# JuliaLinearAlgebra/IterativeSolvers.jl

Hardware: AMD Instinct MI355X
Metric: cg_iters_per_sec (higher is better)
Workload: dtype f64; 1 GPU; cg! on 256^3 3D 7-point Laplacian (test/laplace_matrix.jl), fp64, hashed rhs, x0 = 0 (BASELINE.json configs[1]); n=16777216, nnz=117047296

## Files before the change

iterativesolvers.jl_amd/csrc/mik_iter.h:

```cpp
#pragma once
#include "mik_internal.h"

template <typename T> struct CgDev {
    T res, prev_res, alpha, beta, dot_uc, rr, tol, rho;
    T beta_rho;
    int done, nhist;
    int x_pending, pad_;
};

struct CgMirror {
    double res, prev_res, tol;
    int done, nhist;
    int tol_valid;
    int range;
    unsigned long long seq;
};

struct mik_cg {
    mik_ctx *ctx = nullptr;
    const mik_csr *A = nullptr;
    int dtype = MIK_F64;
    int64_t n = 0;
    void *x = nullptr, *u = nullptr, *r = nullptr, *c = nullptr;
    const void *b = nullptr, *diag = nullptr;
    mik_mul_fn op_mul = nullptr;
    void *op_user = nullptr;
    mik_ldiv_fn pl_fn = nullptr;
    void *pl_user = nullptr;
    void *dev = nullptr;
    void *fin = nullptr;
    void *hist = nullptr;
    int64_t hist_cap = 0;
    void *seg_spmv = nullptr;
    void *seg_vec = nullptr;
    void *seg_vec2 = nullptr;
    bool pcg_fused = false;
    double residual = 0, prev_residual = 1, tol = 0;
    int64_t maxiter = 0, mv_products = 0;
    CgMirror *mirror = nullptr;
    unsigned long long seq = 0;
    bool dev_done = false;
    bool head_ahead = false;
    bool fuse_x = false;
    int profile = 0;
    std::vector<hipEvent_t> ev;
    std::vector<int> ev_kind;
    size_t ev_used = 0;
    double kern_ms[3] = {0, 0, 0};
    int64_t kern_launches[3] = {0, 0, 0};
};

#ifdef __HIPCC__
constexpr int MIK_FIN_WGS = MIK_FIN_THREADS / 64;
template <typename T> struct FinScratch { T ws[MIK_FIN_WGS]; unsigned ticket; };

template <typename T> __device__ __forceinline__ bool level2_sum_spread(const T *__restrict__ S, int64_t m, FinScratch<T> *fs, T &tot)
{
    const int w = blockIdx.x, lane = threadIdx.x;
    T acc = T(0);
    int64_t j = 64 * (int64_t)w + lane;
    for (; j + 63 * (int64_t)MIK_FIN_THREADS < m; j += 64 * (int64_t)MIK_FIN_THREADS) {
        T v[64];
#pragma unroll
        for (int q = 0; q < 64; ++q) v[q] = S[j + q * (int64_t)MIK_FIN_THREADS];
#pragma unroll
        for (int q = 0; q < 64; ++q) acc = acc + v[q];
    }
    for (; j + 15 * (int64_t)MIK_FIN_THREADS < m; j += 16 * (int64_t)MIK_FIN_THREADS) {
        T v[16];
#pragma unroll
        for (int q = 0; q < 16; ++q) v[q] = S[j + q * (int64_t)MIK_FIN_THREADS];
#pragma unroll
        for (int q = 0; q < 16; ++q) acc = acc + v[q];
    }
    for (; j + 7 * (int64_t)MIK_FIN_THREADS < m; j += 8 * (int64_t)MIK_FIN_THREADS) {
        T v[8];
#pragma unroll
        for (int q = 0; q < 8; ++q) v[q] = S[j + q * (int64_t)MIK_FIN_THREADS];
#pragma unroll
        for (int q = 0; q < 8; ++q) acc = acc + v[q];
    }
    for (; j < m; j += MIK_FIN_THREADS) acc = acc + S[j];
    acc = wave_tree(acc);
    bool last = false;
    if (lane == 0) {
        __hip_atomic_store(&fs->ws[w], acc, __ATOMIC_RELAXED, __HIP_MEMORY_SCOPE_AGENT);
        asm volatile("s_waitcnt vmcnt(0)" ::: "memory");
        const unsigned tk = __hip_atomic_fetch_add(&fs->ticket, 1u, __ATOMIC_RELAXED, __HIP_MEMORY_SCOPE_AGENT);
        if (tk == (unsigned)gridDim.x - 1u) {
            T t = __hip_atomic_load(&fs->ws[0], __ATOMIC_RELAXED, __HIP_MEMORY_SCOPE_AGENT);
#pragma unroll
            for (int q = 1; q < MIK_FIN_WGS; ++q) t = t + __hip_atomic_load(&fs->ws[q], __ATOMIC_RELAXED, __HIP_MEMORY_SCOPE_AGENT);
            __hip_atomic_store(&fs->ticket, 0u, __ATOMIC_RELAXED, __HIP_MEMORY_SCOPE_AGENT);
            tot = t;
            last = true;
        }
    }
    return last;
}

template <typename T>
__device__ __forceinline__ void cgd_close_step(CgDev<T> *d, T tot, T *__restrict__ hist, long long it_next, long long maxiter, CgMirror *mirror,
                                               unsigned long long seq, int hist_index, int fuse_x)
{
    if (fuse_x) d->x_pending = 1;
    if (!mik_nrm_in_range(tot)) {
        d->done = 1; mirror->done = 0; mirror->nhist = hist_index; mirror->range = 1;
        __hip_atomic_store(&mirror->seq, seq, __ATOMIC_RELEASE, __HIP_MEMORY_SCOPE_SYSTEM);
        return;
    }
    const T prev = d->res;
    const T res = mik_sqrt(tot);
    d->rr = tot; d->prev_res = prev; d->res = res;
    d->beta = (res * res) / (prev * prev);
    hist[hist_index] = res;
    const int nh = hist_index + 1;
    const int dn = (it_next >= maxiter || res <= d->tol) ? 1 : 0;
    if (dn) d->done = 1;
    mirror->res = (double)res; mirror->prev_res = (double)prev; mirror->done = dn; mirror->nhist = nh;
    __hip_atomic_store(&mirror->seq, seq, __ATOMIC_RELEASE, __HIP_MEMORY_SCOPE_SYSTEM);
}
#endif

int cg_wait_mirror(mik_cg *it);

template <class R> static int cg_run_batch(R &rk, int64_t iteration, int64_t max_steps, bool ahead_ok, double *residuals, int64_t *steps_done)
// ... 83 lines not shown
```

iterativesolvers.jl_amd/csrc/mik_kernels.h:

```cpp
#pragma once
#include <algorithm>

#include "mik_internal.h"

#ifdef __HIPCC__


template <typename T, bool VEC, typename Op>
__global__ __launch_bounds__(MIK_BLOCK) void k_map(int64_t n, int64_t nseg, Op op, T *__restrict__ seg_out,
                                                    const int *__restrict__ done)
{
    if (done && *done) return;
    constexpr int W = VT<T>::W;
    constexpr int L = MIK_RED_L;
    constexpr int64_t SEG = (int64_t)MIK_BLOCK * W * L;
    __shared__ T lds4[4];
    for (int64_t s = blockIdx.x; s < nseg; s += gridDim.x) {
        const int64_t base = s * SEG + (int64_t)W * threadIdx.x;
        T acc = T(0);
#pragma unroll
        for (int l = 0; l < L; ++l) {
            const int64_t i = base + (int64_t)l * MIK_BLOCK * W;
            if (VEC && i + W <= n) {
                op.apply_vec(i, acc);
// ... 469 lines not shown
        auto xv = vload<T>(x + i); auto yv = vload<T>(y + i);
#pragma unroll
        for (int e = 0; e < VT<T>::W; ++e) { el<T>(xv, e) = el<T>(xv, e) * a; el<T>(yv, e) = el<T>(yv, e) * b; }
        vstore(x + i, xv); vstore(y + i, yv);
    }
};

template <typename T> struct OpQmrUpdate {
    static constexpr bool REDUCE = false;
    const T *__restrict__ v; const T *p_curr; const T *p_prev; T *p_out; T *__restrict__ x; T neg_h1, neg_h0, inv, g;
    __device__ __forceinline__ void apply(int64_t i, T &) const
    {
        T p = v[i];
        if (p_curr) { T t = neg_h1 * p_curr[i]; p = p + t; }
        if (p_prev) { T t = neg_h0 * p_prev[i]; p = p + t; }
        p = p * inv;
        p_out[i] = p;
        T t = g * p; x[i] = x[i] + t;
    }
    __device__ __forceinline__ void apply_vec(int64_t i, T &) const
    {
        constexpr int W = VT<T>::W;
        auto pv = vload(v + i); auto xv = vload_nt<T>(x + i);
        if (p_curr) {
            auto cv = vload(p_curr + i);
#pragma unroll
            for (int e = 0; e < W; ++e) { T t = neg_h1 * el<T>(cv, e); el<T>(pv, e) = el<T>(pv, e) + t; }
        }
        if (p_prev) {
            auto qv = vload(p_prev + i);
#pragma unroll
            for (int e = 0; e < W; ++e) { T t = neg_h0 * el<T>(qv, e); el<T>(pv, e) = el<T>(pv, e) + t; }
        }
#pragma unroll
        for (int e = 0; e < W; ++e) { el<T>(pv, e) = el<T>(pv, e) * inv; T t = g * el<T>(pv, e); el<T>(xv, e) = el<T>(xv, e) + t; }
        vstore(p_out + i, pv); vstore_nt(x + i, xv);
    }
};

template <typename T> struct OpXpbyX {
    static constexpr bool REDUCE = false;
    const T *__restrict__ r; T *__restrict__ u; T *__restrict__ x; Coef<T> beta, alpha;
    const int *__restrict__ done; const int *__restrict__ pending; int nt = 0;
    __device__ __forceinline__ void apply(int64_t i, T &) const
    {
        const int dn = *done, pd = *pending;
        if (dn && !pd) return;
        const T uo = u[i];
        if (pd) { T t = alpha.get() * uo; x[i] = x[i] + t; }
        if (!dn) { T t = beta.get() * uo; u[i] = r[i] + t; }
    }
    __device__ __forceinline__ void apply_vec(int64_t i, T &) const
    {
        const int dn = *done, pd = *pending;
        if (dn && !pd) return;
        auto uv = (nt & 2) ? vload_nt<T>(u + i) : vload<T>(u + i);
        if (pd) {
            const T a = alpha.get();
            auto xv = (nt & 8) ? vload_nt<T>(x + i) : vload<T>(x + i);
#pragma unroll
            for (int e = 0; e < VT<T>::W; ++e) { T t = a * el<T>(uv, e); el<T>(xv, e) = el<T>(xv, e) + t; }
            if (nt & 8) vstore_nt(x + i, xv); else vstore(x + i, xv);
        }
        if (!dn) {
            const T b = beta.get();
            auto rv = (nt & 1) ? vload_nt(r + i) : vload(r + i);
#pragma unroll
            for (int e = 0; e < VT<T>::W; ++e) { T t = b * el<T>(uv, e); el<T>(uv, e) = el<T>(rv, e) + t; }
            if (nt & 4) vstore_nt(u + i, uv); else vstore(u + i, uv);
        }
    }
};

template <typename T> struct CoefAlphaRanks {
    const T *all; int nranks; const T *res;
    __device__ __forceinline__ T get() const
    {
        T tot = all[0];
        for (int p = 1; p < nranks; ++p) tot = tot + all[p];
        const T r = *res;
        return (r * r) / tot;
    }
};
template <typename T, typename C = Coef<T>> struct OpCgUpdateR {
    static constexpr bool REDUCE = true;
    T *__restrict__ r; const T *__restrict__ c; C alpha; int nt = 0;
    __device__ __forceinline__ void apply(int64_t i, T &acc) const
    {
        T s = alpha.get() * c[i]; T rn = r[i] - s; r[i] = rn;
        T p = rn * rn; acc = acc + p;
    }
    __device__ __forceinline__ void apply_vec(int64_t i, T &acc) const
    {
        const T a = alpha.get();
        auto rv = (nt & 8) ? vload_nt<T>(r + i) : vload<T>(r + i);
        auto cv = (nt & 2) ? vload_nt(c + i) : vload(c + i);
#pragma unroll
        for (int e = 0; e < VT<T>::W; ++e) { T s = a * el<T>(cv, e); el<T>(rv, e) = el<T>(rv, e) - s; }
        if (nt & 16) vstore_nt(r + i, rv); else vstore(r + i, rv);
#pragma unroll
        for (int e = 0; e < VT<T>::W; ++e) { T p = el<T>(rv, e) * el<T>(rv, e); acc = acc + p; }
    }
};

template <typename T> struct OpPcgUpdateR {
    static constexpr bool REDUCE = true;
    T *__restrict__ r; T *__restrict__ c; const T *__restrict__ d; Coef<T> alpha; int nt = 0;
    __device__ __forceinline__ void apply(int64_t i, T &a1, T &a2) const
    {
        T s = alpha.get() * c[i]; T rn = r[i] - s; r[i] = rn;
        T p = rn * rn; a1 = a1 + p;
        T v = rn / d[i]; c[i] = v;
        T q = v * rn; a2 = a2 + q;
    }
    __device__ __forceinline__ void apply_vec(int64_t i, T &a1, T &a2) const
    {
        const T a = alpha.get();
        auto rv = (nt & 8) ? vload_nt<T>(r + i) : vload<T>(r + i);
        auto cv = (nt & 64) ? vload_nt<T>(c + i) : vload<T>(c + i);
        auto dv = vload_nt(d + i);
#pragma unroll
        for (int e = 0; e < VT<T>::W; ++e) { T s = a * el<T>(cv, e); el<T>(rv, e) = el<T>(rv, e) - s; }
        if (nt & 16) vstore_nt(r + i, rv); else vstore(r + i, rv);
#pragma unroll
        for (int e = 0; e < VT<T>::W; ++e) { T p = el<T>(rv, e) * el<T>(rv, e); a1 = a1 + p; }
#pragma unroll
        for (int e = 0; e < VT<T>::W; ++e) el<T>(cv, e) = el<T>(rv, e) / el<T>(dv, e);
        if (nt & 32) vstore_nt(c + i, cv); else vstore(c + i, cv);
#pragma unroll
        for (int e = 0; e < VT<T>::W; ++e) { T q = el<T>(cv, e) * el<T>(rv, e); a2 = a2 + q; }
    }
};

template <typename T> struct OpXFlush {
    static constexpr bool REDUCE = false;
    const T *__restrict__ u; T *__restrict__ x; Coef<T> alpha; const int *__restrict__ pending;
    __device__ __forceinline__ void apply(int64_t i, T &) const
    {
        if (!*pending) return;
        T t = alpha.get() * u[i]; x[i] = x[i] + t;
    }
    __device__ __forceinline__ void apply_vec(int64_t i, T &) const
    {
        if (!*pending) return;
        const T a = alpha.get();
        auto uv = vload(u + i); auto xv = vload<T>(x + i);
#pragma unroll
        for (int e = 0; e < VT<T>::W; ++e) { T t = a * el<T>(uv, e); el<T>(xv, e) = el<T>(xv, e) + t; }
        vstore(x + i, xv);
    }
};

template <typename T> struct OpAxpy {
    static constexpr bool REDUCE = false;
    const T *__restrict__ x; T *__restrict__ y; Coef<T> alpha;
    __device__ __forceinline__ void apply(int64_t i, T &) const { T t = alpha.get() * x[i]; y[i] = y[i] + t; }
    __device__ __forceinline__ void apply_vec(int64_t i, T &) const
    {
        const T a = alpha.get();
        auto xv = vload(x + i); auto yv = vload<T>(y + i);
#pragma unroll
        for (int e = 0; e < VT<T>::W; ++e) { T t = a * el<T>(xv, e); el<T>(yv, e) = el<T>(yv, e) + t; }
        vstore(y + i, yv);
    }
};

template <typename T> struct OpBicgU {
    static constexpr bool REDUCE = false;
    T *__restrict__ us; int64_t ldu; const T *__restrict__ rs; int64_t ldr; int ncols; Coef<T> neg_beta;
    int nt = 0;
    __device__ __forceinline__ void apply(int64_t i, T &) const
    {
        const T b = neg_beta.get();
        for (int q = 0; q < ncols; ++q) { T *u = us + q * ldu; T t = b * u[i]; u[i] = rs[q * ldr + i] + t; }
    }
    __device__ __forceinline__ void apply_vec(int64_t i, T &) const
    {
        const T b = neg_beta.get();
        for (int q = 0; q < ncols; ++q) {
            T *u = us + q * ldu;
            auto xv = (nt & 1) ? vload_nt(rs + q * ldr + i) : vload(rs + q * ldr + i);
            auto yv = (nt & 1) ? vload_nt<T>(u + i) : vload<T>(u + i);
#pragma unroll
            for (int e = 0; e < VT<T>::W; ++e) { T t = b * el<T>(yv, e); el<T>(yv, e) = el<T>(xv, e) + t; }
            if (q + 1 < ncols ? (nt & 2) : (nt & 4)) vstore_nt(u + i, yv); else vstore(u + i, yv);
        }
// ... 988 lines not shown
```

iterativesolvers.jl_amd/csrc/mik_krylov.hip:

```cpp
#include <algorithm>
#include <cfloat>
#include <cstddef>
#include <cmath>
#include <map>
#include <new>
#include <tuple>

#include "mik_kernels.h"
#include "mik_mgs_res.h"
#include "mik_iter.h"
#include "mik_mail.h"

template <typename T>
int mik_spmv_launch(mik_ctx *ctx, const mik_csr *A, const T *x, T *y, bool fuse_dot, T *seg_out, const int *done);
template <typename T>
int mik_spmv_launch_range(mik_ctx *ctx, const mik_csr *A, const T *x, T *y, bool fuse_dot, T *seg_out, const int *done, int rb_begin,
                          int rb_count);
template <typename T>
int mik_spmv_launch_outside(mik_ctx *ctx, const mik_csr *A, const T *x, T *y, bool fuse_dot, T *seg_out, const int *done, int skip_begin, int skip_end);
bool mik_spmv_can_split(const mik_csr *A);
bool mik_spmv_is_light(const mik_csr *A);



// ... 377 lines not shown
        for (int q = 0; q < 16; ++q) { a1 = a1 + v[q]; a2 = a2 + z[q]; }
    }
    for (; j < m; j += MIK_FIN_THREADS) { a1 = a1 + S1[j]; a2 = a2 + S2[j]; }
    a1 = wave_tree(a1);
    a2 = wave_tree(a2);
    bool last = false;
    if (lane == 0) {
        __hip_atomic_store(&fs->ws[w], a1, __ATOMIC_RELAXED, __HIP_MEMORY_SCOPE_AGENT);
        __hip_atomic_store(&fs->ws2[w], a2, __ATOMIC_RELAXED, __HIP_MEMORY_SCOPE_AGENT);
        asm volatile("s_waitcnt vmcnt(0)" ::: "memory");
        const unsigned tk = __hip_atomic_fetch_add(&fs->ticket, 1u, __ATOMIC_RELAXED, __HIP_MEMORY_SCOPE_AGENT);
        if (tk == (unsigned)gridDim.x - 1u) {
            T t = __hip_atomic_load(&fs->ws[0], __ATOMIC_RELAXED, __HIP_MEMORY_SCOPE_AGENT);
            T z = __hip_atomic_load(&fs->ws2[0], __ATOMIC_RELAXED, __HIP_MEMORY_SCOPE_AGENT);
#pragma unroll
            for (int q = 1; q < MIK_FIN_WGS; ++q) {
                t = t + __hip_atomic_load(&fs->ws[q], __ATOMIC_RELAXED, __HIP_MEMORY_SCOPE_AGENT);
                z = z + __hip_atomic_load(&fs->ws2[q], __ATOMIC_RELAXED, __HIP_MEMORY_SCOPE_AGENT);
            }
            __hip_atomic_store(&fs->ticket, 0u, __ATOMIC_RELAXED, __HIP_MEMORY_SCOPE_AGENT);
            tot1 = t; tot2 = z;
            last = true;
        }
    }
    return last;
}

template <typename T> __device__ __forceinline__ void cg_init_scalars(CgDev<T> *d, T tot, T res, T reltol, T abstol, long long maxiter)
{
    const T a = reltol * res;
    d->rr = tot;
    d->res = res;
    d->prev_res = T(1);
    d->rho = T(1);
    d->tol = a > abstol ? a : abstol;
    d->beta = (res * res) / (T(1) * T(1));
    d->alpha = T(0);
    d->dot_uc = T(0);
    d->done = (0 >= maxiter || res <= d->tol) ? 1 : 0;
    d->nhist = 0;
}

template <typename T>
__global__ __launch_bounds__(MIK_FIN_THREADS) void k_cg_fin_init(const T *__restrict__ S, int64_t m, CgDev<T> *d, T reltol, T abstol,
                                                                 long long maxiter)
{
    __shared__ T lds16[16];
    T tot = level2_sum(S, m, lds16);
    if (threadIdx.x == 0) { cg_init_scalars(d, tot, mik_sqrt(tot), reltol, abstol, maxiter); d->x_pending = 0; }
}

template <typename T> __global__ void k_cg_set_init(CgDev<T> *d, T res, T reltol, T abstol, long long maxiter)
{
    cg_init_scalars(d, res * res, res, reltol, abstol, maxiter);
    d->x_pending = 0;
}

template <typename T>
__global__ __launch_bounds__(64) void k_cg_fin_alpha(const T *__restrict__ S, int64_t m, CgDev<T> *d, int pcg, FinScratch<T> *fs)
{
    if (blockIdx.x == 0 && threadIdx.x == 0) d->x_pending = 0;
    if (d->done) return;
    T tot;
    if (level2_sum_spread(S, m, fs, tot)) {
        d->dot_uc = tot;
        const T num = pcg ? d->rho : d->res * d->res;
        d->alpha = num / tot;
    }
}

template <typename T>
__global__ __launch_bounds__(64) void k_cg_fin_rho(const T *__restrict__ S, int64_t m, CgDev<T> *d, FinScratch<T> *fs)
{
    if (d->done) return;
    T tot;
    if (level2_sum_spread(S, m, fs, tot)) {
        const T rho_prev = d->rho;
        d->rho = tot;
        d->beta = tot / rho_prev;
    }
}

template <typename T>
__device__ __forceinline__ void cg_res_scalars(CgDev<T> *d, T tot, T res, T *__restrict__ hist, long long it_next, long long maxiter,
                                               CgMirror *mirror, unsigned long long seq, int hist_index, int pcg_fused = 0)
{
    const T prev = d->res;
    d->rr = tot;
    d->prev_res = prev;
    d->res = res;
    d->beta = pcg_fused ? d->beta_rho : (res * res) / (prev * prev);
    hist[hist_index] = res;
    const int dn = (it_next >= maxiter || res <= d->tol) ? 1 : 0;
    if (dn) d->done = 1;
    mirror->res = (double)res;
    mirror->prev_res = (double)prev;
    mirror->done = dn;
    mirror->nhist = hist_index + 1;
    __hip_atomic_store(&mirror->seq, seq, __ATOMIC_RELEASE, __HIP_MEMORY_SCOPE_SYSTEM);
}

template <typename T>
__global__ __launch_bounds__(64) void k_cg_fin_res(const T *__restrict__ S, int64_t m, CgDev<T> *d, T *__restrict__ hist,
                                                    long long it_next, long long maxiter, CgMirror *mirror,
                                                    unsigned long long seq, int hist_index, FinScratch<T> *fs, int fuse_x)
{
    if (d->done) {
        if (blockIdx.x == 0 && threadIdx.x == 0) __hip_atomic_store(&mirror->seq, seq, __ATOMIC_RELEASE, __HIP_MEMORY_SCOPE_SYSTEM);
        return;
    }
    T tot;
    if (level2_sum_spread(S, m, fs, tot)) {
        if (fuse_x) d->x_pending = 1;
        if (!mik_nrm_in_range(tot)) {
            d->done = 1;
            mirror->done = 0;
            mirror->nhist = hist_index;
            mirror->range = 1;
            __hip_atomic_store(&mirror->seq, seq, __ATOMIC_RELEASE, __HIP_MEMORY_SCOPE_SYSTEM);
            return;
        }
        cg_res_scalars(d, tot, mik_sqrt(tot), hist, it_next, maxiter, mirror, seq, hist_index);
    }
}

template <typename T>
__global__ void k_cg_fix_res(CgDev<T> *d, T res, T *__restrict__ hist, long long it_next, long long maxiter, CgMirror *mirror,
                             unsigned long long seq, int hist_index, int pcg_fused = 0)
{
    d->done = 0;
    mirror->range = 0;
    cg_res_scalars(d, res * res, res, hist, it_next, maxiter, mirror, seq, hist_index, pcg_fused);
}

template <typename T>
__global__ __launch_bounds__(64) void k_cg_fin_res2(const T *__restrict__ S1, const T *__restrict__ S2, int64_t m, CgDev<T> *d, T *__restrict__ hist,
                                                     long long it_next, long long maxiter, CgMirror *mirror, unsigned long long seq, int hist_index,
                                                     FinScratch2<T> *fs)
{
    if (d->done) {
        if (blockIdx.x == 0 && threadIdx.x == 0) __hip_atomic_store(&mirror->seq, seq, __ATOMIC_RELEASE, __HIP_MEMORY_SCOPE_SYSTEM);
        return;
    }
    T tot, tot2;
    if (level2_sum_spread2(S1, S2, m, fs, tot, tot2)) {
        d->x_pending = 1;
        const T rho_prev = d->rho;
        d->rho = tot2;
        d->beta_rho = tot2 / rho_prev;
        if (!mik_nrm_in_range(tot)) {
            d->done = 1;
            mirror->done = 0;
            mirror->nhist = hist_index;
            mirror->range = 1;
            __hip_atomic_store(&mirror->seq, seq, __ATOMIC_RELEASE, __HIP_MEMORY_SCOPE_SYSTEM);
            return;
        }
        cg_res_scalars(d, tot, mik_sqrt(tot), hist, it_next, maxiter, mirror, seq, hist_index, 1);
    }
}

static int cg_profile_collect(mik_cg *it)
{
    size_t i = 0;
    for (; i + 1 < it->ev_used; i += 2) {
        if (hipEventQuery(it->ev[i + 1]) != hipSuccess) { (void)hipGetLastError(); break; }
        float ms = 0.f;
        const int kind = it->ev_kind[i / 2];
        if (hipEventElapsedTime(&ms, it->ev[i], it->ev[i + 1]) == hipSuccess) { it->kern_ms[kind] += ms; it->kern_launches[kind] += 1; }
    }
    size_t keep = 0;
    for (size_t j = i; j + 1 < it->ev_used; j += 2, keep += 2) {
        std::swap(it->ev[keep], it->ev[j]);
        std::swap(it->ev[keep + 1], it->ev[j + 1]);
        it->ev_kind[keep / 2] = it->ev_kind[j / 2];
    }
    it->ev_used = keep;
    return MIK_OK;
}

static void cg_profile_flush(mik_cg *it)
{
    if (!it->ev_used) return;
    (void)hipStreamSynchronize(it->ctx->stream);
    (void)cg_profile_collect(it);
}

struct CgProfileScope {
    mik_cg *it; bool on;
    CgProfileScope(mik_cg *it_, int kind) : it(it_), on(it_->profile == 2 || (it_->profile == 1 && kind == 0))
    {
        if (!on) return;
        if (it->ev_used + 2 > it->ev.size()) {
            hipEvent_t a, b;
            if (hipEventCreate(&a) != hipSuccess || hipEventCreate(&b) != hipSuccess) { on = false; return; }
            it->ev.push_back(a); it->ev.push_back(b);
            it->ev_kind.push_back(0);
        }
        it->ev_kind[it->ev_used / 2] = kind;
        (void)hipEventRecord(it->ev[it->ev_used], it->ctx->stream);
    }
    ~CgProfileScope()
    {
        if (!on) return;
        (void)hipEventRecord(it->ev[it->ev_used + 1], it->ctx->stream);
        it->ev_used += 2;
    }
};

static inline int cg_stream_hints(const mik_ctx *ctx, bool fused_x = false, const mik_csr *A = nullptr)
{
    (void)ctx;
    return fused_x ? (mik_spmv_is_light(A) ? 248 : 121) : 57;
}


static inline int cg_sweep_u_hints(const mik_cg *it) { return it->fuse_x ? cg_stream_hints(it->ctx, true, it->A) & 15 : cg_stream_hints(it->ctx) & 7; }

template <typename T> static int cg_sweep_u(mik_cg *it, const T *src, int64_t lo, int64_t len, bool vec, int hints)
{
    CgDev<T> *d = (CgDev<T> *)it->dev;
    T *x = (T *)it->x, *u = (T *)it->u;
    if (it->fuse_x) {
        OpXpbyX<T> op{src + lo, u + lo, x + lo, coef_ptr<T>(&d->beta), coef_ptr<T>(&d->alpha), &d->done, &d->x_pending, hints};
        return launch_map<T>(it->ctx, len, op, vec, (T *)nullptr, (const int *)nullptr);
    }
    OpXpby<T> op{src + lo, u + lo, coef_ptr<T>(&d->beta), hints};
    return launch_map<T>(it->ctx, len, op, vec, (T *)nullptr, &d->done);
}

template <typename T, typename C> static int cg_update_xr(mik_cg *it, C alpha, bool vec)
{
    CgDev<T> *d = (CgDev<T> *)it->dev;
    T *x = (T *)it->x, *u = (T *)it->u, *r = (T *)it->r, *c = (T *)it->c;
    if (it->fuse_x) {
        OpCgUpdateR<T, C> up{r, c, alpha, cg_stream_hints(it->ctx, true, it->A) >> 3};
        return launch_map<T>(it->ctx, it->n, up, vec, (T *)it->seg_vec, &d->done);
    }
    if constexpr (std::is_same<C, Coef<T>>::value) {
        OpCgUpdate<T> up{x, r, u, c, alpha, cg_stream_hints(it->ctx) >> 3};
        return launch_map<T>(it->ctx, it->n, up, vec, (T *)it->seg_vec, &d->done);
    }
    return mik_fail(it->ctx, MIK_ERR_INVALID, "cg: alpha formed inside the sweep needs the x update on the next sweep over u");
}

template <typename T> __global__ void k_cg_clear_pending(CgDev<T> *d) { d->x_pending = 0; }

template <typename T> static int cg_flush_x(mik_cg *it)
{
    mik_ctx *ctx = it->ctx;
    CgDev<T> *d = (CgDev<T> *)it->dev;
    T *x = (T *)it->x, *u = (T *)it->u;
    OpXFlush<T> op{u, x, coef_ptr<T>(&d->alpha), &d->x_pending};
    MIK_TRY((launch_map<T>(ctx, it->n, op, mik_aligned16(x) && mik_aligned16(u), (T *)nullptr, (const int *)nullptr)));
    hipLaunchKernelGGL((k_cg_clear_pending<T>), dim3(1), dim3(1), 0, ctx->stream, d);
    MIK_LAUNCH_CHECK(ctx);
    return MIK_OK;
}

template <typename T> static int cg_init_residual(mik_cg *it, const T *x0, bool vec)
{
    mik_ctx *ctx = it->ctx;
    T *c = (T *)it->c;
    it->mv_products = x0 ? 1 : 0;
    if (x0) {
        if (it->A) MIK_TRY(mik_spmv_launch<T>(ctx, it->A, x0, c, false, nullptr, nullptr));
        else if (it->op_mul(it->op_user, x0, c) != 0) return mik_fail(ctx, MIK_ERR_CALLBACK, "cg: the operator callback failed");
    }
    OpSubNrm<T> op{(const T *)it->b, x0 ? c : nullptr, (T *)it->r};
    return launch_map<T>(ctx, it->n, op, vec, (T *)it->seg_vec, nullptr);
}

template <typename T> static int cg_enqueue_head(mik_cg *it)
{
    mik_ctx *ctx = it->ctx;
    CgDev<T> *d = (CgDev<T> *)it->dev;
    const int *done = &d->done;
    const int64_t n = it->n, nseg = mik_nseg<T>(n);
    T *x = (T *)it->x, *u = (T *)it->u, *r = (T *)it->r, *c = (T *)it->c;
    const bool vec = mik_aligned16(x) && mik_aligned16(u) && mik_aligned16(r) && mik_aligned16(c) && (!it->diag || mik_aligned16(it->diag));
    const int pcg = (it->diag || it->pl_fn) ? 1 : 0;
    if (it->pcg_fused) {
    } else if (it->diag) {
        OpJacobiDot<T> pj{r, (const T *)it->diag, c, cg_stream_hints(ctx) != 0};
        MIK_TRY((launch_map<T>(ctx, n, pj, vec, (T *)it->seg_vec, done)));
    } else if (it->pl_fn) {
        if (it->pl_fn(it->pl_user, c, r) != 0) return mik_fail(ctx, MIK_ERR_CALLBACK, "cg: the preconditioner callback failed");
        OpDot<T> dcr{c, r};
        MIK_TRY((launch_map<T>(ctx, n, dcr, vec, (T *)it->seg_vec, done)));
    }
    if (pcg && !it->pcg_fused) {
        hipLaunchKernelGGL((k_cg_fin_rho<T>), dim3(MIK_FIN_WGS), dim3(64), 0, ctx->stream, (const T *)it->seg_vec, nseg, d, (FinScratch<T> *)it->fin);
        MIK_LAUNCH_CHECK(ctx);
    }
    {
        CgProfileScope ps(it, 1);
        const int pcg_hints = it->fuse_x ? (cg_stream_hints(ctx, true, it->A) & 8) | 1 : cg_stream_hints(ctx) & 1;
        MIK_TRY(cg_sweep_u<T>(it, pcg ? c : r, 0, n, vec, pcg ? pcg_hints : cg_sweep_u_hints(it)));
    }
    if (it->A) {
        CgProfileScope ps(it, 0);
        MIK_TRY(mik_spmv_launch<T>(ctx, it->A, u, c, true, (T *)it->seg_spmv, done));
    } else {
        if (it->op_mul(it->op_user, u, c) != 0) return mik_fail(ctx, MIK_ERR_CALLBACK, "cg: the operator callback failed");
        OpDot<T> duc{u, c};
        MIK_TRY((launch_map<T>(ctx, n, duc, vec, (T *)it->seg_vec, done)));
    }
    hipLaunchKernelGGL((k_cg_fin_alpha<T>), dim3(MIK_FIN_WGS), dim3(64), 0, ctx->stream, (const T *)(it->A ? it->seg_spmv : it->seg_vec), it->A ? mik_spmv_nwg(n) : nseg,
                       d, pcg, (FinScratch<T> *)it->fin);
    MIK_LAUNCH_CHECK(ctx);
    return MIK_OK;
}

template <typename T> static int cg_enqueue_tail(mik_cg *it, long long it_next, int hist_index)
{
    mik_ctx *ctx = it->ctx;
    CgDev<T> *d = (CgDev<T> *)it->dev;
    const int *done = &d->done;
    const int64_t n = it->n, nseg = mik_nseg<T>(n);
    T *x = (T *)it->x, *u = (T *)it->u, *r = (T *)it->r, *c = (T *)it->c;
    const bool vec = mik_aligned16(x) && mik_aligned16(u) && mik_aligned16(r) && mik_aligned16(c) && (!it->diag || mik_aligned16(it->diag));
    if (it->pcg_fused) {
        {
            CgProfileScope ps(it, 2);
            OpPcgUpdateR<T> up{r, c, (const T *)it->diag, coef_ptr<T>(&d->alpha), 120};
            MIK_TRY((launch_map2<T>(ctx, n, up, vec, (T *)it->seg_vec, (T *)it->seg_vec2, done)));
        }
        it->seq += 1;
        hipLaunchKernelGGL((k_cg_fin_res2<T>), dim3(MIK_FIN_WGS), dim3(64), 0, ctx->stream, (const T *)it->seg_vec, (const T *)it->seg_vec2, nseg, d, (T *)it->hist,
                           it_next, (long long)it->maxiter, it->mirror, it->seq, hist_index, (FinScratch2<T> *)((unsigned char *)it->fin + 512));
        MIK_LAUNCH_CHECK(ctx);
        return MIK_OK;
    }
    {
        CgProfileScope ps(it, 2);
        MIK_TRY(cg_update_xr<T>(it, coef_ptr<T>(&d->alpha), vec));
    }
    it->seq += 1;
    hipLaunchKernelGGL((k_cg_fin_res<T>), dim3(MIK_FIN_WGS), dim3(64), 0, ctx->stream, (const T *)it->seg_vec, nseg, d, (T *)it->hist,
                       it_next, (long long)it->maxiter, it->mirror, it->seq, hist_index, (FinScratch<T> *)it->fin, it->fuse_x ? 1 : 0);
    MIK_LAUNCH_CHECK(ctx);
    return MIK_OK;
}

int cg_wait_mirror(mik_cg *it)
{
    volatile unsigned long long *p = &it->mirror->seq;
    const unsigned long long want = it->seq;
    for (unsigned long long spins = 0;; ++spins) {
        if (__atomic_load_n((const unsigned long long *)p, __ATOMIC_ACQUIRE) == want) return MIK_OK;
        if ((spins & 0xFFFFF) == 0xFFFFF) {
            hipError_t e = hipStreamQuery(it->ctx->stream);
            if (e == hipSuccess) {
                if (__atomic_load_n((const unsigned long long *)p, __ATOMIC_ACQUIRE) == want) return MIK_OK;
                return mik_fail(it->ctx, MIK_ERR_HIP, "cg: stream idle but step %llu was never published", want);
            }
            if (e != hipErrorNotReady) return mik_fail(it->ctx, MIK_ERR_HIP, "cg: %s while waiting for a step", hipGetErrorString(e));
        }
#if defined(__x86_64__)
        __builtin_ia32_pause();
#endif
    }
}

template <typename T> static int cg_fetch_state(mik_cg *it, CgDev<T> *host)
{
    mik_ctx *ctx = it->ctx;
    MIK_HIP(ctx, hipMemcpyAsync(ctx->coef_host, it->dev, sizeof(CgDev<T>), hipMemcpyDeviceToHost, ctx->stream));
    MIK_HIP(ctx, hipStreamSynchronize(ctx->stream));
    memcpy(host, ctx->coef_host, sizeof(CgDev<T>));
    return MIK_OK;
}

template <typename T>
static int cg_init_impl(mik_cg *it, double abstol, double reltol, int initially_zero)
{
    mik_ctx *ctx = it->ctx;
    const int64_t n = it->n, nseg = mik_nseg<T>(n);
    T *u = (T *)it->u, *r = (T *)it->r, *c = (T *)it->c;
    OpFill<T> z{u, T(0)};
    MIK_TRY((launch_map<T>(ctx, n, z, mik_aligned16(u), (T *)nullptr, nullptr)));
    const bool vec = mik_aligned16(r) && mik_aligned16(it->b) && mik_aligned16(c);
    MIK_TRY(cg_init_residual<T>(it, initially_zero ? nullptr : (const T *)it->x, vec));
    hipLaunchKernelGGL((k_cg_fin_init<T>), dim3(1), dim3(MIK_FIN_THREADS), 0, ctx->stream, (const T *)it->seg_vec, nseg,
                       (CgDev<T> *)it->dev, (T)reltol, (T)abstol, (long long)it->maxiter);
    MIK_LAUNCH_CHECK(ctx);
    CgDev<T> h;
    MIK_TRY(cg_fetch_state<T>(it, &h));
    if (!mik_nrm_in_range(h.rr)) {
        T res;
        MIK_TRY(mik_safe_norm_slow<T>(ctx, n, r, &res));
        hipLaunchKernelGGL((k_cg_set_init<T>), dim3(1), dim3(1), 0, ctx->stream, (CgDev<T> *)it->dev, res, (T)reltol, (T)abstol, (long long)it->maxiter);
        MIK_LAUNCH_CHECK(ctx);
        MIK_TRY(cg_fetch_state<T>(it, &h));
    }
    it->residual = (double)h.res;
    it->prev_residual = (double)h.prev_res;
    it->tol = (double)h.tol;
    it->dev_done = h.done != 0;
    if (it->pcg_fused) {
        OpJacobiDot<T> pj{r, (const T *)it->diag, c, 0};
        MIK_TRY((launch_map<T>(ctx, n, pj, vec && mik_aligned16(it->diag), (T *)it->seg_vec, (const int *)nullptr)));
        hipLaunchKernelGGL((k_cg_fin_rho<T>), dim3(MIK_FIN_WGS), dim3(64), 0, ctx->stream, (const T *)it->seg_vec, nseg, (CgDev<T> *)it->dev, (FinScratch<T> *)it->fin);
        MIK_LAUNCH_CHECK(ctx);
    }
    return MIK_OK;
}

static int cg_create_common(mik_ctx *ctx, const mik_csr *A, int dtype, int64_t n, mik_mul_fn op_mul, void *op_user, const void *jacobi_diag,
                            mik_ldiv_fn pl_fn, void *pl_user, void *x, const void *b, void *u, void *r, void *c, double abstol, double reltol,
                            int64_t maxiter, int initially_zero, mik_cg **out)
{
    if (n && (!x || !b || !u || !r || !c)) return mik_fail(ctx, MIK_ERR_INVALID, "mik_cg_create: NULL vector");
    mik_cg *it = new (std::nothrow) mik_cg();
    if (!it) return mik_fail(ctx, MIK_ERR_NOMEM, "mik_cg_create: host allocation failed");
    it->ctx = ctx; it->A = A; it->dtype = dtype; it->n = n;
    it->op_mul = op_mul; it->op_user = op_user; it->pl_fn = pl_fn; it->pl_user = pl_user;
    it->x = x; it->b = b; it->u = u; it->r = r; it->c = c; it->diag = jacobi_diag;
    it->maxiter = maxiter;
    it->fuse_x = A != nullptr && !pl_fn && (ctx->tuning[MIK_KNOB_CG_STEP] & 1) == 0;
    it->pcg_fused = it->fuse_x && jacobi_diag != nullptr && (ctx->tuning[MIK_KNOB_CG_STEP] & 2) == 0;
    const size_t es = mik_dtype_size(dtype);
    const int64_t nseg = dtype == MIK_F64 ? mik_nseg<double>(n) : mik_nseg<float>(n);
    const int64_t nb = mik_spmv_nwg(n);
    hipError_t e;
    (void)hipSetDevice(ctx->device);
    if ((e = hipMalloc(&it->dev, 256)) != hipSuccess || (e = hipMalloc(&it->fin, 1024)) != hipSuccess ||
        (e = hipMemsetAsync(it->fin, 0, 1024, ctx->stream)) != hipSuccess ||
        (it->pcg_fused && (e = hipMalloc(&it->seg_vec2, es * (size_t)std::max<int64_t>(nseg, 1))) != hipSuccess) || (e = hipMalloc(&it->seg_spmv, es * (size_t)std::max<int64_t>(nb, 1))) != hipSuccess ||
        (e = hipMalloc(&it->seg_vec, es * (size_t)std::max<int64_t>(nseg, 1))) != hipSuccess ||
        (e = hipMalloc(&it->hist, es * 64)) != hipSuccess) {
        mik_cg_destroy(it);
        return mik_fail(ctx, MIK_ERR_NOMEM, "mik_cg_create: hipMalloc: %s", hipGetErrorString(e));
    }
    it->hist_cap = 64;
    if ((e = hipHostMalloc((void **)&it->mirror, sizeof(CgMirror), hipHostMallocMapped | hipHostMallocCoherent)) != hipSuccess) {
        mik_cg_destroy(it);
        return mik_fail(ctx, MIK_ERR_NOMEM, "mik_cg_create: hipHostMalloc: %s", hipGetErrorString(e));
    }
    memset(it->mirror, 0, sizeof(CgMirror));
    int rc = dtype == MIK_F64 ? cg_init_impl<double>(it, abstol, reltol, initially_zero)
                              : cg_init_impl<float>(it, abstol, reltol, initially_zero);
    if (rc) { mik_cg_destroy(it); return rc; }
    *out = it;
    return MIK_OK;
}

extern "C" int mik_cg_create(mik_ctx *ctx, const mik_csr *A, void *x, const void *b, void *u, void *r, void *c,
                             const void *jacobi_diag, double abstol, double reltol, int64_t maxiter, int initially_zero,
                             mik_cg **out)
{
    if (!ctx || !out) return MIK_ERR_INVALID;
    *out = nullptr;
    if (!A || A->n_rows != A->n_cols) return mik_fail(ctx, MIK_ERR_MISMATCH, "mik_cg_create: A must be square");
    return cg_create_common(ctx, A, A->dtype, A->n_rows, nullptr, nullptr, jacobi_diag, nullptr, nullptr, x, b, u, r, c, abstol, reltol, maxiter,
                            initially_zero, out);
}

static int resolve_operator(mik_ctx *ctx, const mik_operator *A, const char *who, const mik_csr **csr, int *dtype, int64_t *n)
{
    if (!A || (!A->csr && !A->mul)) return mik_fail(ctx, MIK_ERR_INVALID, "%s: the operator needs a csr handle or a mul callback", who);
    if (A->csr) {
        if (A->csr->n_rows != A->csr->n_cols) return mik_fail(ctx, MIK_ERR_MISMATCH, "%s: A must be square", who);
        *csr = A->csr; *dtype = A->csr->dtype; *n = A->csr->n_rows;
        return MIK_OK;
    }
    if ((A->dtype != MIK_F64 && A->dtype != MIK_F32) || A->n < 0) return mik_fail(ctx, MIK_ERR_INVALID, "%s: bad dtype / size of the callback operator", who);
    *csr = nullptr; *dtype = A->dtype; *n = A->n;
    return MIK_OK;
}

extern "C" int mik_cg_create_op(mik_ctx *ctx, const mik_operator *A, const mik_precond *Pl, void *x, const void *b, void *u, void *r, void *c,
                                double abstol, double reltol, int64_t maxiter, int initially_zero, mik_cg **out)
{
    if (!ctx || !out) return MIK_ERR_INVALID;
    *out = nullptr;
    const mik_csr *csr = nullptr;
    int dtype = MIK_F64;
    int64_t n = 0;
    MIK_TRY(resolve_operator(ctx, A, "mik_cg_create_op", &csr, &dtype, &n));
    if (Pl && Pl->diag && Pl->ldiv) return mik_fail(ctx, MIK_ERR_INVALID, "mik_cg_create_op: Pl has both a diagonal and a callback");
    return cg_create_common(ctx, csr, dtype, n, csr ? nullptr : A->mul, A->user, Pl ? Pl->diag : nullptr, Pl ? Pl->ldiv : nullptr,
                            Pl ? Pl->user : nullptr, x, b, u, r, c, abstol, reltol, maxiter, initially_zero, out);
}

extern "C" int mik_cg_destroy(mik_cg *it)
{
    if (!it) return MIK_OK;
    if (it->ctx) (void)hipStreamSynchronize(it->ctx->stream);
    if (it->dev) (void)hipFree(it->dev);
    if (it->fin) (void)hipFree(it->fin);
    if (it->hist) (void)hipFree(it->hist);
    if (it->seg_spmv) (void)hipFree(it->seg_spmv);
    if (it->seg_vec) (void)hipFree(it->seg_vec);
    if (it->seg_vec2) (void)hipFree(it->seg_vec2);
    for (hipEvent_t e : it->ev) (void)hipEventDestroy(e);
    if (it->mirror) (void)hipHostFree(it->mirror);
    delete it;
    return MIK_OK;
}

template <typename T> struct CgLocal {
    mik_cg *it;
    T res = T(0);
    mik_cg &base() { return *it; }
    int head(int64_t) { return cg_enqueue_head<T>(it); }
    int tail(int64_t iteration, int64_t j) { return cg_enqueue_tail<T>(it, (long long)(iteration + 1), (int)j); }
    int flush_x() { return cg_flush_x<T>(it); }
    int wait(CgMirror *m) { MIK_TRY(cg_wait_mirror(it)); *m = *it->mirror; return MIK_OK; }
    int clear_pending() { return MIK_OK; }
    int scaled_norm() { return mik_safe_norm_slow<T>(it->ctx, it->n, (const T *)it->r, &res); }
    int close_frozen(int64_t it_next, int hist_index)
    {
        it->seq += 1;
        hipLaunchKernelGGL((k_cg_fix_res<T>), dim3(1), dim3(1), 0, it->ctx->stream, (CgDev<T> *)it->dev, res, (T *)it->hist, (long long)it_next,
                           (long long)it->maxiter, it->mirror, it->seq, hist_index, it->pcg_fused ? 1 : 0);
        MIK_LAUNCH_CHECK(it->ctx);
        return MIK_OK;
    }
    int collect(const CgMirror &m, double *, double *, double *residuals, int64_t, int64_t *steps_done)
    {
        mik_ctx *ctx = it->ctx;
        const int64_t nd = m.nhist;
        if (nd == 1) {
            if (residuals) residuals[0] = m.res;
        } else if (nd > 1) {
            std::vector<T> tmp((size_t)nd);
            MIK_HIP(ctx, hipMemcpyAsync(tmp.data(), it->hist, sizeof(T) * (size_t)nd, hipMemcpyDeviceToHost, ctx->stream));
            MIK_HIP(ctx, hipStreamSynchronize(ctx->stream));
            if (residuals) for (int64_t j = 0; j < nd; ++j) residuals[j] = (double)tmp[j];
        }
        if (nd > 0) {
            it->residual = m.res;
            it->prev_residual = m.prev_res;
        }
        it->dev_done = m.done != 0;
        it->mv_products += nd;
        *steps_done = nd;
        if (it->profile) cg_profile_collect(it);
        return MIK_OK;
    }
};

template <typename T>
static int cg_iterate_many_impl(mik_cg *it, int64_t iteration, int64_t max_steps, double *residuals, int64_t *steps_done)
{
    mik_ctx *ctx = it->ctx;
    *steps_done = 0;
    if (max_steps <= 0 || iteration >= it->maxiter || it->residual <= it->tol) return MIK_OK;
    max_steps = std::min(max_steps, it->maxiter - iteration);
    if ((it->op_mul || it->pl_fn) && max_steps > 1) {
        int64_t total = 0;
        for (int64_t j = 0; j < max_steps; ++j) {
            int64_t nd1 = 0;
            double res1 = 0;
            MIK_TRY(cg_iterate_many_impl<T>(it, iteration + j, 1, &res1, &nd1));
            if (nd1 == 0) break;
            if (residuals) residuals[total] = res1;
            total += 1;
        }
        *steps_done = total;
        return MIK_OK;
    }
    if (max_steps > it->hist_cap) {
        MIK_HIP(ctx, hipStreamSynchronize(ctx->stream));
        MIK_HIP(ctx, hipFree(it->hist));
        it->hist = nullptr;
        MIK_HIP(ctx, hipMalloc(&it->hist, sizeof(T) * (size_t)max_steps));
        it->hist_cap = max_steps;
    }
    it->mirror->nhist = 0;
    it->mirror->range = 0;
    if (it->dev_done) MIK_HIP(ctx, hipMemsetAsync(&((CgDev<T> *)it->dev)->done, 0, sizeof(int), ctx->stream));
    const bool ahead_ok = ctx->tuning[MIK_KNOB_NO_LOOKAHEAD] == 0 && !it->op_mul && !it->pl_fn && iteration + max_steps < it->maxiter;
    CgLocal<T> rk{it};
    return cg_run_batch(rk, iteration, max_steps, ahead_ok, residuals, steps_done);
}

extern "C" int mik_cg_iterate_many(mik_cg *it, int64_t iteration, int64_t max_steps, double *residuals, int64_t *steps_done)
{
    if (!it || !steps_done || iteration < 0) return MIK_ERR_INVALID;
    return it->dtype == MIK_F64 ? cg_iterate_many_impl<double>(it, iteration, max_steps, residuals, steps_done)
                                : cg_iterate_many_impl<float>(it, iteration, max_steps, residuals, steps_done);
}

extern "C" int mik_cg_iterate(mik_cg *it, int64_t iteration, double *residual, int *done)
{
    if (!it || !done) return MIK_ERR_INVALID;
    int64_t nd = 0;
    double res = 0;
    int rc = mik_cg_iterate_many(it, iteration, 1, &res, &nd);
    if (rc) return rc;
// ... 1109 lines not shown
```

Baseline: 2175 iters/s.

## Fold residual reduction finalize into next head sweep with persistent-grid fold kernels

```diff
diff --git a/iterativesolvers.jl_amd/csrc/mik_iter.h b/iterativesolvers.jl_amd/csrc/mik_iter.h
--- a/iterativesolvers.jl_amd/csrc/mik_iter.h
+++ b/iterativesolvers.jl_amd/csrc/mik_iter.h
@@ -6,6 +6,8 @@
     T beta_rho;
     int done, nhist;
     int x_pending, pad_;
+    T snap_res;
+    int snap_done, pad2_;
 };
 
 struct CgMirror {
@@ -42,6 +44,10 @@
     bool dev_done = false;
     bool head_ahead = false;
     bool fuse_x = false;
+    bool fold = false;
+    bool res_open = false;
+    long long open_it_next = 0;
+    int open_hist_index = 0;
     int profile = 0;
     std::vector<hipEvent_t> ev;
     std::vector<int> ev_kind;
diff --git a/iterativesolvers.jl_amd/csrc/mik_kernels.h b/iterativesolvers.jl_amd/csrc/mik_kernels.h
--- a/iterativesolvers.jl_amd/csrc/mik_kernels.h
+++ b/iterativesolvers.jl_amd/csrc/mik_kernels.h
@@ -575,7 +575,11 @@
         return (r * r) / tot;
     }
 };
-template <typename T, typename C = Coef<T>> struct OpCgUpdateR {
+template <typename T> struct CoefReg {
+    T v;
+    __device__ __forceinline__ T get() const { return v; }
+};
+template <typename T, typename C = Coef<T>, int NTC = -1> struct OpCgUpdateR {
     static constexpr bool REDUCE = true;
     T *__restrict__ r; const T *__restrict__ c; C alpha; int nt = 0;
     __device__ __forceinline__ void apply(int64_t i, T &acc) const
@@ -583,18 +587,201 @@
         T s = alpha.get() * c[i]; T rn = r[i] - s; r[i] = rn;
         T p = rn * rn; acc = acc + p;
     }
-    __device__ __forceinline__ void apply_vec(int64_t i, T &acc) const
-    {
+    struct Regs { typename VT<T>::vec rv, cv; };
+    static constexpr int FOLD_DEPTH = 3;
+    __device__ __forceinline__ void load_vec(int64_t i, Regs &g) const
+    {
+        const int NT = NTC >= 0 ? NTC : nt;
+        g.rv = (NT & 8) ? vload_nt<T>(r + i) : vload<T>(r + i);
+        g.cv = (NT & 2) ? vload_nt(c + i) : vload(c + i);
+    }
+    __device__ __forceinline__ void compute_vec(int64_t i, Regs &g, T &acc) const
+    {
+        const int NT = NTC >= 0 ? NTC : nt;
         const T a = alpha.get();
-        auto rv = (nt & 8) ? vload_nt<T>(r + i) : vload<T>(r + i);
-        auto cv = (nt & 2) ? vload_nt(c + i) : vload(c + i);
-#pragma unroll
-        for (int e = 0; e < VT<T>::W; ++e) { T s = a * el<T>(cv, e); el<T>(rv, e) = el<T>(rv, e) - s; }
-        if (nt & 16) vstore_nt(r + i, rv); else vstore(r + i, rv);
-#pragma unroll
-        for (int e = 0; e < VT<T>::W; ++e) { T p = el<T>(rv, e) * el<T>(rv, e); acc = acc + p; }
-    }
-};
+#pragma unroll
+        for (int e = 0; e < VT<T>::W; ++e) { T s = a * el<T>(g.cv, e); el<T>(g.rv, e) = el<T>(g.rv, e) - s; }
+        if (NT & 16) vstore_nt(r + i, g.rv); else vstore(r + i, g.rv);
+#pragma unroll
+        for (int e = 0; e < VT<T>::W; ++e) { T p = el<T>(g.rv, e) * el<T>(g.rv, e); acc = acc + p; }
+    }
+    __device__ __forceinline__ void apply_vec(int64_t i, T &acc) const { Regs g; load_vec(i, g); compute_vec(i, g, acc); }
+};
+
+template <typename T, int NT> struct OpXpbyXLocal {
+    static constexpr bool REDUCE = false;
+    const T *__restrict__ r; T *__restrict__ u; T *__restrict__ x;
+    T beta = T(0), alpha = T(0); int dn = 0, pd = 0;
+    __device__ __forceinline__ void apply(int64_t i, T &) const
+    {
+        const T uo = u[i];
+        if (pd) { T t = alpha * uo; x[i] = x[i] + t; }
+        if (!dn) { T t = beta * uo; u[i] = r[i] + t; }
+    }
+    struct Regs { typename VT<T>::vec uv, xv, rv; };
+    static constexpr int FOLD_DEPTH = 2;
+    __device__ __forceinline__ void load_vec(int64_t i, Regs &g) const
+    {
+        g.uv = (NT & 2) ? vload_nt<T>(u + i) : vload<T>(u + i);
+        g.xv = (NT & 8) ? vload_nt<T>(x + i) : vload<T>(x + i);
+        g.rv = (NT & 1) ? vload_nt(r + i) : vload(r + i);
+    }
+    __device__ __forceinline__ void compute_vec(int64_t i, Regs &g, T &) const
+    {
+        if (pd) {
+#pragma unroll
+            for (int e = 0; e < VT<T>::W; ++e) { T t = alpha * el<T>(g.uv, e); el<T>(g.xv, e) = el<T>(g.xv, e) + t; }
+            if (NT & 8) vstore_nt(x + i, g.xv); else vstore(x + i, g.xv);
+        }
+        if (!dn) {
+#pragma unroll
+            for (int e = 0; e < VT<T>::W; ++e) { T t = beta * el<T>(g.uv, e); el<T>(g.uv, e) = el<T>(g.rv, e) + t; }
+            if (NT & 4) vstore_nt(u + i, g.uv); else vstore(u + i, g.uv);
+        }
+    }
+};
+
+constexpr int MIK_FOLD = MIK_FIN_THREADS;
+template <typename T> static inline int mik_nfold(int64_t n) { return (int)std::min<int64_t>(mik_nseg<T>(n), MIK_FOLD); }
+
+template <typename T, int D> __device__ __forceinline__ void block_trees_256(const T (&acc)[D], T (&tot)[D], T *ldsw)
+{
+    const int lane = threadIdx.x & 63, w = threadIdx.x >> 6;
+#pragma unroll
+    for (int k = 0; k < D; ++k) {
+        const T v = wave_tree(acc[k]);
+        if (lane == 0) ldsw[4 * k + w] = v;
+    }
+    __syncthreads();
+#pragma unroll
+    for (int k = 0; k < D; ++k) {
+        tot[k] = T(0);
+        if (threadIdx.x == 0) {
+            T t = ldsw[4 * k];
+            t = t + ldsw[4 * k + 1];
+            t = t + ldsw[4 * k + 2];
+            t = t + ldsw[4 * k + 3];
+            tot[k] = t;
+        }
+    }
+    __syncthreads();
+}
+
+template <typename T, bool VEC, typename Op> struct SegShare {
+    static constexpr int W = VT<T>::W, L = MIK_RED_L;
+    static constexpr int64_t SEG = (int64_t)MIK_BLOCK * W * L;
+    typename Op::Regs rg[L];
+    bool whole;
+    __device__ __forceinline__ void load_whole(const Op &op, int64_t s)
+    {
+        whole = true;
+        const int64_t base = s * SEG + (int64_t)W * threadIdx.x;
+#pragma unroll
+        for (int l = 0; l < L; ++l) op.load_vec(base + (int64_t)l * MIK_BLOCK * W, rg[l]);
+    }
+    __device__ __forceinline__ T compute_whole(const Op &op, int64_t s)
+    {
+        const int64_t base = s * SEG + (int64_t)W * threadIdx.x;
+        T acc = T(0);
+#pragma unroll
+        for (int l = 0; l < L; ++l) op.compute_vec(base + (int64_t)l * MIK_BLOCK * W, rg[l], acc);
+        return acc;
+    }
+    __device__ __forceinline__ void load(const Op &op, int64_t n, int64_t s)
+    {
+        whole = VEC && (s + 1) * SEG <= n;
+        if (whole) load_whole(op, s);
+    }
+    __device__ __forceinline__ T compute(const Op &op, int64_t n, int64_t s)
+    {
+        if (whole) return compute_whole(op, s);
+        const int64_t base = s * SEG + (int64_t)W * threadIdx.x;
+        T acc = T(0);
+#pragma unroll
+        for (int l = 0; l < L; ++l) {
+            const int64_t i = base + (int64_t)l * MIK_BLOCK * W;
+            if (VEC && i + W <= n) {
+                typename Op::Regs g;
+                op.load_vec(i, g);
+                op.compute_vec(i, g, acc);
+            } else {
+#pragma unroll
+                for (int e = 0; e < W; ++e)
+                    if (i + e < n) op.apply(i + e, acc);
+            }
+        }
+        return acc;
+    }
+};
+
+template <typename T, bool VEC, typename Op, typename Pro>
+__global__ __launch_bounds__(MIK_BLOCK, 4) void k_map_fold(int64_t n, int64_t nseg, Op op, Pro pro, T *__restrict__ fold_out)
+{
+    constexpr int D = Op::FOLD_DEPTH;
+    __shared__ T lds16[16];
+    __shared__ T ldsw[4 * D];
+    const int64_t G = gridDim.x;
+    const int64_t nwhole = VEC ? n / SegShare<T, VEC, Op>::SEG : 0;
+    SegShare<T, VEC, Op> sh[D];
+    int64_t s = blockIdx.x;
+    const bool steady = s + (D - 1) * G < nwhole;
+    if (steady) {
+#pragma unroll
+        for (int k = 0; k < D; ++k) sh[k].load_whole(op, s + k * G);
+    } else {
+#pragma unroll
+        for (int k = 0; k < D; ++k)
+            if (s + k * G < nseg) sh[k].load(op, n, s + k * G);
+    }
+    if (!pro(op, lds16)) return;
+    T vacc = T(0);
+    if (steady) {
+        for (; s + (2 * D - 1) * G < nwhole; s += D * G) {
+            T acc[D], tot[D];
+#pragma unroll
+            for (int k = 0; k < D; ++k) {
+                acc[k] = sh[k].compute_whole(op, s + k * G);
+                sh[k].load_whole(op, s + (k + D) * G);
+            }
+            if (Op::REDUCE) {
+                block_trees_256<T, D>(acc, tot, ldsw);
+#pragma unroll
+                for (int k = 0; k < D; ++k) vacc = vacc + tot[k];
+            }
+        }
+    }
+    for (; s < nseg; s += D * G) {
+        T acc[D], tot[D];
+#pragma unroll
+        for (int k = 0; k < D; ++k) {
+            const int64_t sk = s + k * G;
+            acc[k] = T(0);
+            if (sk < nseg) {
+                acc[k] = sh[k].compute(op, n, sk);
+                if (sk + D * G < nseg) sh[k].load(op, n, sk + D * G);
+            }
+        }
+        if (Op::REDUCE) {
+            block_trees_256<T, D>(acc, tot, ldsw);
+#pragma unroll
+            for (int k = 0; k < D; ++k)
+                if (s + k * G < nseg) vacc = vacc + tot[k];
+        }
+    }
+    if (Op::REDUCE && threadIdx.x == 0) fold_out[blockIdx.x] = vacc;
+}
+
+template <typename T, typename Op, typename Pro>
+static inline int launch_map_fold(mik_ctx *ctx, int64_t n, Op op, Pro pro, bool vec, T *fold_out)
+{
+    const int64_t nseg = mik_nseg<T>(n);
+    if (nseg == 0) return MIK_OK;
+    const int grid = mik_nfold<T>(n);
+    if (vec) hipLaunchKernelGGL((k_map_fold<T, true, Op, Pro>), dim3(grid), dim3(MIK_BLOCK), 0, ctx->stream, n, nseg, op, pro, fold_out);
+    else hipLaunchKernelGGL((k_map_fold<T, false, Op, Pro>), dim3(grid), dim3(MIK_BLOCK), 0, ctx->stream, n, nseg, op, pro, fold_out);
+    MIK_LAUNCH_CHECK(ctx);
+    return MIK_OK;
+}
 
 template <typename T> struct OpPcgUpdateR {
     static constexpr bool REDUCE = true;
diff --git a/iterativesolvers.jl_amd/csrc/mik_krylov.hip b/iterativesolvers.jl_amd/csrc/mik_krylov.hip
--- a/iterativesolvers.jl_amd/csrc/mik_krylov.hip
+++ b/iterativesolvers.jl_amd/csrc/mik_krylov.hip
@@ -483,10 +483,9 @@
 }
 
 template <typename T>
-__device__ __forceinline__ void cg_res_scalars(CgDev<T> *d, T tot, T res, T *__restrict__ hist, long long it_next, long long maxiter,
-                                               CgMirror *mirror, unsigned long long seq, int hist_index, int pcg_fused = 0)
-{
-    const T prev = d->res;
+__device__ __forceinline__ void cg_res_scalars_from(CgDev<T> *d, T prev, T tot, T res, T *__restrict__ hist, long long it_next, long long maxiter,
+                                                    CgMirror *mirror, unsigned long long seq, int hist_index, int pcg_fused = 0)
+{
     d->rr = tot;
     d->prev_res = prev;
     d->res = res;
@@ -500,6 +499,12 @@
     mirror->nhist = hist_index + 1;
     __hip_atomic_store(&mirror->seq, seq, __ATOMIC_RELEASE, __HIP_MEMORY_SCOPE_SYSTEM);
 }
+template <typename T>
+__device__ __forceinline__ void cg_res_scalars(CgDev<T> *d, T tot, T res, T *__restrict__ hist, long long it_next, long long maxiter,
+                                               CgMirror *mirror, unsigned long long seq, int hist_index, int pcg_fused = 0)
+{
+    cg_res_scalars_from(d, d->res, tot, res, hist, it_next, maxiter, mirror, seq, hist_index, pcg_fused);
+}
 
 template <typename T>
 __global__ __launch_bounds__(64) void k_cg_fin_res(const T *__restrict__ S, int64_t m, CgDev<T> *d, T *__restrict__ hist,
@@ -533,6 +538,56 @@
     mirror->range = 0;
     cg_res_scalars(d, res * res, res, hist, it_next, maxiter, mirror, seq, hist_index, pcg_fused);
 }
+
+template <typename T> struct CgTailPro {
+    CgDev<T> *d;
+    template <typename Op> __device__ __forceinline__ bool operator()(Op &op, T *) const
+    {
+        op.alpha.v = d->alpha;
+        const int dn = d->done;
+        if (blockIdx.x == 0 && threadIdx.x == 0) { d->snap_done = dn; d->snap_res = d->res; }
+        return !dn;
+    }
+};
+
+template <typename T> struct CgHeadPro {
+    const T *__restrict__ V; int m;
+    CgDev<T> *d; T *__restrict__ hist; long long it_next, maxiter; CgMirror *mirror; unsigned long long seq; int hist_index;
+    template <typename Op> __device__ __forceinline__ bool operator()(Op &op, T *lds16) const
+    {
+        const bool lead = blockIdx.x == 0 && threadIdx.x == 0;
+        op.alpha = d->alpha;
+        op.beta = T(0);
+        if (d->snap_done) {
+            if (lead) __hip_atomic_store(&mirror->seq, seq, __ATOMIC_RELEASE, __HIP_MEMORY_SCOPE_SYSTEM);
+            op.dn = 1;
+            op.pd = d->x_pending;
+            return op.pd != 0;
+        }
+        const T tot = block_level2_256(V, m, lds16);
+        op.pd = 1;
+        if (!mik_nrm_in_range(tot)) {
+            if (lead) {
+                d->x_pending = 1;
+                d->done = 1;
+                mirror->done = 0;
+                mirror->nhist = hist_index;
+                mirror->range = 1;
+                __hip_atomic_store(&mirror->seq, seq, __ATOMIC_RELEASE, __HIP_MEMORY_SCOPE_SYSTEM);
+            }
+            op.dn = 1;
+            return true;
+        }
+        const T res = mik_sqrt(tot), prev = d->snap_res;
+        op.beta = (res * res) / (prev * prev);
+        op.dn = (it_next >= maxiter || res <= d->tol) ? 1 : 0;
+        if (lead) {
+            d->x_pending = 1;
+            cg_res_scalars_from(d, prev, tot, res, hist, it_next, maxiter, mirror, seq, hist_index);
+        }
+        return true;
+    }
+};
 
 template <typename T>
 __global__ __launch_bounds__(64) void k_cg_fin_res2(const T *__restrict__ S1, const T *__restrict__ S2, int64_t m, CgDev<T> *d, T *__restrict__ hist,
@@ -609,10 +664,11 @@
     }
 };
 
+constexpr int cg_fused_hints(bool light) { return light ? 248 : 121; }
 static inline int cg_stream_hints(const mik_ctx *ctx, bool fused_x = false, const mik_csr *A = nullptr)
 {
     (void)ctx;
-    return fused_x ? (mik_spmv_is_light(A) ? 248 : 121) : 57;
+    return fused_x ? cg_fused_hints(mik_spmv_is_light(A)) : 57;
 }
 
 
@@ -694,7 +750,13 @@
         hipLaunchKernelGGL((k_cg_fin_rho<T>), dim3(MIK_FIN_WGS), dim3(64), 0, ctx->stream, (const T *)it->seg_vec, nseg, d, (FinScratch<T> *)it->fin);
         MIK_LAUNCH_CHECK(ctx);
     }
-    {
+    if (it->res_open) {
+        CgProfileScope ps(it, 1);
+        CgHeadPro<T> pro{(const T *)it->seg_vec, mik_nfold<T>(n), d, (T *)it->hist, it->open_it_next, (long long)it->maxiter, it->mirror, it->seq, it->open_hist_index};
+        it->res_open = false;
+        if (mik_spmv_is_light(it->A)) { MIK_TRY((launch_map_fold<T>(ctx, n, OpXpbyXLocal<T, (cg_fused_hints(true) & 15)>{r, u, x}, pro, vec, (T *)nullptr))); }
+        else { MIK_TRY((launch_map_fold<T>(ctx, n, OpXpbyXLocal<T, (cg_fused_hints(false) & 15)>{r, u, x}, pro, vec, (T *)nullptr))); }
+    } else {
         CgProfileScope ps(it, 1);
         const int pcg_hints = it->fuse_x ? (cg_stream_hints(ctx, true, it->A) & 8) | 1 : cg_stream_hints(ctx) & 1;
         MIK_TRY(cg_sweep_u<T>(it, pcg ? c : r, 0, n, vec, pcg ? pcg_hints : cg_sweep_u_hints(it)));
@@ -733,6 +795,16 @@
         MIK_LAUNCH_CHECK(ctx);
         return MIK_OK;
     }
+    if (it->fold) {
+        CgProfileScope ps(it, 2);
+        if (mik_spmv_is_light(it->A)) { MIK_TRY((launch_map_fold<T>(ctx, n, OpCgUpdateR<T, CoefReg<T>, (cg_fused_hints(true) >> 3)>{r, c, CoefReg<T>{T(0)}}, CgTailPro<T>{d}, vec, (T *)it->seg_vec))); }
+        else { MIK_TRY((launch_map_fold<T>(ctx, n, OpCgUpdateR<T, CoefReg<T>, (cg_fused_hints(false) >> 3)>{r, c, CoefReg<T>{T(0)}}, CgTailPro<T>{d}, vec, (T *)it->seg_vec))); }
+        it->seq += 1;
+        it->res_open = true;
+        it->open_it_next = it_next;
+        it->open_hist_index = hist_index;
+        return MIK_OK;
+    }
     {
         CgProfileScope ps(it, 2);
         MIK_TRY(cg_update_xr<T>(it, coef_ptr<T>(&d->alpha), vec));
@@ -740,6 +812,17 @@
     it->seq += 1;
     hipLaunchKernelGGL((k_cg_fin_res<T>), dim3(MIK_FIN_WGS), dim3(64), 0, ctx->stream, (const T *)it->seg_vec, nseg, d, (T *)it->hist,
                        it_next, (long long)it->maxiter, it->mirror, it->seq, hist_index, (FinScratch<T> *)it->fin, it->fuse_x ? 1 : 0);
+    MIK_LAUNCH_CHECK(ctx);
+    return MIK_OK;
+}
+
+template <typename T> static int cg_close_tail(mik_cg *it)
+{
+    if (!it->res_open) return MIK_OK;
+    mik_ctx *ctx = it->ctx;
+    it->res_open = false;
+    hipLaunchKernelGGL((k_cg_fin_res<T>), dim3(MIK_FIN_WGS), dim3(64), 0, ctx->stream, (const T *)it->seg_vec, (int64_t)mik_nfold<T>(it->n), (CgDev<T> *)it->dev, (T *)it->hist,
+                       it->open_it_next, (long long)it->maxiter, it->mirror, it->seq, it->open_hist_index, (FinScratch<T> *)it->fin, 1);
     MIK_LAUNCH_CHECK(ctx);
     return MIK_OK;
 }
@@ -821,6 +904,7 @@
     it->maxiter = maxiter;
     it->fuse_x = A != nullptr && !pl_fn && (ctx->tuning[MIK_KNOB_CG_STEP] & 1) == 0;
     it->pcg_fused = it->fuse_x && jacobi_diag != nullptr && (ctx->tuning[MIK_KNOB_CG_STEP] & 2) == 0;
+    it->fold = it->fuse_x && !jacobi_diag && n > 0 && (ctx->tuning[MIK_KNOB_CG_STEP] & 16) == 0;
     const size_t es = mik_dtype_size(dtype);
     const int64_t nseg = dtype == MIK_F64 ? mik_nseg<double>(n) : mik_nseg<float>(n);
     const int64_t nb = mik_spmv_nwg(n);
@@ -907,8 +991,8 @@
     mik_cg &base() { return *it; }
     int head(int64_t) { return cg_enqueue_head<T>(it); }
     int tail(int64_t iteration, int64_t j) { return cg_enqueue_tail<T>(it, (long long)(iteration + 1), (int)j); }
-    int flush_x() { return cg_flush_x<T>(it); }
-    int wait(CgMirror *m) { MIK_TRY(cg_wait_mirror(it)); *m = *it->mirror; return MIK_OK; }
+    int flush_x() { MIK_TRY(cg_close_tail<T>(it)); return cg_flush_x<T>(it); }
+    int wait(CgMirror *m) { MIK_TRY(cg_close_tail<T>(it)); MIK_TRY(cg_wait_mirror(it)); *m = *it->mirror; return MIK_OK; }
     int clear_pending() { return MIK_OK; }
     int scaled_norm() { return mik_safe_norm_slow<T>(it->ctx, it->n, (const T *)it->r, &res); }
     int close_frozen(int64_t it_next, int hist_index)
```

Result: slower. 2141 iters/s (-1.6%).
